# lonelycorn/mvSLAM

Measured on AMD Instinct MI355X. Metric: image-pairs/sec (2k kp, 50k RANSAC hyp), higher is better.
Workload: dtype f64; 1 GPU; 512 independent synthetic 640x480 pairs per GPU, 2000 keypoints (256-bit descriptors), 50000 8-point hypotheses per pair, full match+RANSAC+decompose+triangulate; pairs_per_gpu=512, keypoints=2000, hypotheses=50000, parallelism=pairs sharded, dp1, streams=2

## Files before the change

### mvslam_amd/csrc/kernels.hip

```cpp
#include <algorithm>
#include "kernels.hpp"

#include "device_math.hpp"
#include "prescreen.hpp"

namespace mvs {

constexpr uint32_t kKeyNone = 0xffffffffu;
__device__ __forceinline__ uint32_t bcnt_acc(uint32_t x, uint32_t acc)
{
    uint32_t r;
    asm("v_bcnt_u32_b32 %0, %1, %2" : "=v"(r) : "v"(x), "v"(acc));
    return r;
}
__device__ __forceinline__ void key_insert(uint32_t &k0, uint32_t &k1, uint32_t k)
{
    uint32_t m;
    asm("v_med3_u32 %0, %1, %2, %3" : "=v"(m) : "v"(k0), "v"(k1), "v"(k));
    k1 = m;
    k0 = min(k0, k);
}

constexpr int kTopkWaves = 16;
constexpr int kTopkTileBytes = 65536;
// ... 1422 lines not shown
            a1 = __builtin_amdgcn_mfma_f32_32x32x16_bf16(A0, Bop[1][0], a1, 0, 0, 0);
            a0 = __builtin_amdgcn_mfma_f32_32x32x16_bf16(A1, Bop[0][1], a0, 0, 0, 0);
            a1 = __builtin_amdgcn_mfma_f32_32x32x16_bf16(A1, Bop[1][1], a1, 0, 0, 0);
            ++ntile;
            if (c0 + p0 >= n1) {
#pragma unroll
                for (int r = 0; r < 16; r += 2) {
                    const f32x2 x0 = {a0[r], a0[r + 1]}, x1 = {a1[r], a1[r + 1]};
                    const f32x2 s0 = pk_mul(x0, x0), s1 = pk_mul(x1, x1);
                    cu[0] = pk_add(cu[0], pk_ind(s0, negH, tuH[0]));
                    cl[0] = pk_add(cl[0], pk_ind(s0, negH, tlH[0]));
                    cu[1] = pk_add(cu[1], pk_ind(s1, negH, tuH[1]));
                    cl[1] = pk_add(cl[1], pk_ind(s1, negH, tlH[1]));
                }
            } else {
                dense_count(a0, negH, tlH[0], cl[0]);
                dense_count(a1, negH, tlH[1], cl[1]);
            }
        }
    }
    const int npad = Mr - M;
    int lbest = -1;
#pragma unroll
    for (int c = 0; c < 2; ++c) {
        int U = (int)(cu[c].x + cu[c].y), L = (int)(cl[c].x + cl[c].y);
        U += __shfl_xor(U, 32);
        L += __shfl_xor(L, 32);
        U -= wave_dead ? 0 : npad;
        L -= lpos[c] ? npad : 0;
        if (half == 0 && on[c]) {
            const size_t rec = (size_t)pair * Hp + h[c];
            if (!PILOT)
                b.hyp_cnt[rec] = ucnt0[c] + U;
            if (!wave_dead)
                lbest = max(lbest, L);
        }
        if (STATS && b.stats) {
            const unsigned long long ma = __ballot(wave_live && half == 0);
            if (lane == 0 && ma)
                atomicAdd(&b.stats[PILOT ? 8 : 5], (unsigned long long)__popcll(ma) * (unsigned long long)(32 * ntile));
        }
    }
#pragma unroll
    for (int o = 32; o > 0; o >>= 1)
        lbest = max(lbest, __shfl_xor(lbest, o));
    if (lane == 0 && lbest >= 0)
        atomicMax(&s_lmax, lbest);
    __syncthreads();
    if (tid == 0 && s_lmax >= 0)
        __hip_atomic_fetch_max(b.bound + pair, s_lmax, __ATOMIC_RELAXED, __HIP_MEMORY_SCOPE_AGENT);
}

constexpr int kFinUpperWg = 4;
constexpr int kFinUpperTest = 2;
constexpr int kFinUpperThreads = 512;
constexpr int kFinUpperChunk = 768;
template <bool STATS>
__global__ __launch_bounds__(kFinUpperThreads) __attribute__((amdgpu_waves_per_eu(4, 8))) void ransac_finish_upper_kernel(BatchDev b,
                                                                                                                       RunParams rp)
{
    extern __shared__ __attribute__((aligned(16))) double s_cpts[];
    const int pair = blockIdx.x, tid = threadIdx.x, lane = tid & 63, w = tid >> 6, col = lane & 31, half = lane >> 5;
    const int M = min(b.M[pair], b.max_kp);
    if (M < 8 || b.mode[pair] != 1)
        return;
    const int n1 = b.dense_n1[pair];
    const int Mr = (M + 31) & ~31;
    if (n1 >= Mr)
        return;
    const int Bnow = __hip_atomic_load(b.bound + pair, __ATOMIC_RELAXED, __HIP_MEMORY_SCOPE_AGENT);
    const int cmin = Bnow - (M - n1);
    const int n_all = b.ccount[pair];
    const int n_list = cmin <= 0 ? n_all : min(n_all, b.cpos[(size_t)pair * kSortBins + min(cmin, min(M, kSortBins - 1))]);
    const int n_batches = (max(n_list - kFinishThreads, 0) + kFinUpperThreads - 1) / kFinUpperThreads;
    if ((int)blockIdx.y >= n_batches)
        return;
    const size_t Hp = (size_t)b.max_groups * kHypPerBlock;
    const uint32_t *clist = b.clist2 + (size_t)pair * Hp;
    uint4 *s_op = reinterpret_cast<uint4 *>(s_cpts);
    uint4 *s_win = s_op + (size_t)kFinUpperChunk * 4 + w * kDenseWin;
    const PairBox bx = load_box(b, pair);
    const float X1 = (float)fmax(dabs(bx.x1lo), dabs(bx.x1hi)) * (1.f + 0x1p-22f);
    const float Y1 = (float)fmax(dabs(bx.y1lo), dabs(bx.y1hi)) * (1.f + 0x1p-22f);
    const float X2 = (float)fmax(dabs(bx.x2lo), dabs(bx.x2hi)) * (1.f + 0x1p-22f);
    const float Y2 = (float)fmax(dabs(bx.y2lo), dabs(bx.y2hi)) * (1.f + 0x1p-22f);
    const double4 *src = reinterpret_cast<const double4 *>(b.pts + (size_t)pair * b.max_kp * 4);
    const v16f zero = {0, 0, 0, 0, 0, 0, 0, 0, 0, 0, 0, 0, 0, 0, 0, 0};
    unsigned long long evals = 0;
    struct Ent {
        int h, u;
        bool have;
        float4 q0, q1, q2;
    };
    auto fetch_h = [&](int batch, Ent &en) __attribute__((always_inline)) {
        const int e = kFinishThreads + batch * kFinUpperThreads + w * 64 + lane;
        en.have = batch < n_batches && e < n_list;
        en.h = (int)clist[en.have ? e : 0];
    };
    auto fetch_rest = [&](Ent &en) __attribute__((always_inline)) {
        const size_t rec = (size_t)pair * Hp + (en.have ? en.h : 0);
        en.u = b.hyp_cnt[rec];
        const float4 *fr4 = reinterpret_cast<const float4 *>(b.hyp_r32 + rec * kHypRec32);
        en.q0 = fr4[0], en.q1 = fr4[1], en.q2 = fr4[2];
    };
    for (int c0 = n1; c0 < Mr; c0 += kFinUpperChunk) {
        const int nc = min(kFinUpperChunk, Mr - c0);
        Ent nxt, nn;
        fetch_h(blockIdx.y, nxt);
        fetch_h(blockIdx.y + gridDim.y, nn);
        fetch_rest(nxt);
        __syncthreads();
        for (int i = tid; i < nc; i += kFinUpperThreads) {
            uint4 o[2][2];
            if (c0 + i < M) {
                const double4 pd = src[c0 + i];
                const float x1 = (float)pd.x, y1 = (float)pd.y, x2 = (float)pd.z, y2 = (float)pd.w;
                const float ph[9] = {x2 * x1, x2 * y1, x2, y2 * x1, y2 * y1, y2, x1, y1, 1.f};
                dense_operands_pk<2>(ph, o);
            } else {
                const float qn = __builtin_nanf("");
                const float ph[9] = {qn, qn, qn, qn, qn, qn, qn, qn, qn};
                dense_operands_pk<2>(ph, o);
            }
            uint4 *q = s_op + (size_t)(i >> 5) * 128 + (i & 31);
            q[0] = o[0][0];
            q[32] = o[0][1];
            q[64] = o[1][0];
            q[96] = o[1][1];
        }
        __syncthreads();
        const int left0 = M - c0;
        for (int batch = blockIdx.y; batch < n_batches; batch += gridDim.y) {
            const Ent cur = nxt;
            nxt.have = nn.have;
            nxt.h = nn.h;
            fetch_rest(nxt);
            fetch_h(batch + 2 * gridDim.y, nn);
            const bool have = cur.have;
            const int h_l = cur.have ? cur.h : 0;
            const size_t rec_l = (size_t)pair * Hp + h_l;
            const int u_l = cur.u;
            const bool on_l = have && !(u_l + left0 < Bnow);
            if (__ballot(on_l) == 0ull)
                continue;
            {
                const float4 q0 = cur.q0, q1 = cur.q1, q2 = cur.q2;
                const float fr[9] = {q0.x, q0.y, q0.z, q0.w, q1.x, q1.y, q1.z, q1.w, q2.x};
                float sc = dense_scale(q2.y, dense_T(fr, X1, Y1, X2, Y2), on_l);
                float big = 0.f;
#pragma unroll
                for (int k = 0; k < 9; ++k)
                    big = fmaxf(big, fabsf(fr[k]));
                sc = (big * sc < 0x1p100f) ? sc : 0.f;
                float Fs[9];
#pragma unroll
                for (int k = 0; k < 9; ++k)
                    Fs[k] = mul_legacy(fr[k], sc);
                uint4 o[2][2];
                dense_operands_pk<1>(Fs, o);
                uint4 *wo = s_win + (lane >> 5) * 128 + (lane & 31);
                wo[0] = o[0][0];
                wo[32] = o[0][1];
                wo[64] = o[1][0];
                wo[96] = o[1][1];
            }
            int u0[2];
            bool on[2];
            v8bf Bop[2][2];
#pragma unroll
            for (int c = 0; c < 2; ++c) {
                u0[c] = __shfl(u_l, 32 * c + col);
                on[c] = __shfl((int)on_l, 32 * c + col) != 0;
                const uint4 *ro = s_win + c * 128 + half * 32 + col;
                Bop[c][0] = __builtin_bit_cast(v8bf, ro[0]);
                Bop[c][1] = __builtin_bit_cast(v8bf, ro[64]);
            }
            uint32_t nn[2] = {0u, 0u};
            const uint4 *qt = s_op + half * 32 + col;
            const int nt = nc >> 5;
            int t = 0;
            for (; t < nt; ++t) {
                if (t > 0 && (t & (kFinUpperTest - 1)) == 0) {
                    bool any = false;
#pragma unroll
                    for (int c = 0; c < 2; ++c) {
                        int U = 16 * t - (int)nn[c];
                        U += __shfl_xor(U, 32);
                        any = any || (on[c] && !(u0[c] + U + (left0 - 32 * t) < Bnow));
                    }
                    if (__ballot(any) == 0ull)
                        break;
                }
                const uint4 *q = qt + (size_t)t * 128;
                const v8bf A0 = __builtin_bit_cast(v8bf, q[0]), A1 = __builtin_bit_cast(v8bf, q[64]);
                v16f a0, a1;
                a0 = __builtin_amdgcn_mfma_f32_32x32x16_bf16(A0, Bop[0][0], zero, 0, 0, 0);
                a1 = __builtin_amdgcn_mfma_f32_32x32x16_bf16(A0, Bop[1][0], zero, 0, 0, 0);
                a0 = __builtin_amdgcn_mfma_f32_32x32x16_bf16(A1, Bop[0][1], a0, 0, 0, 0);
                a1 = __builtin_amdgcn_mfma_f32_32x32x16_bf16(A1, Bop[1][1], a1, 0, 0, 0);
                nn[0] += (uint32_t)__builtin_popcount(dense_collect(a0) & 0x55555555u);
                nn[1] += (uint32_t)__builtin_popcount(dense_collect(a1) & 0x55555555u);
            }
            int Uc[2];
#pragma unroll
            for (int c = 0; c < 2; ++c) {
                Uc[c] = 16 * t - (int)nn[c];
                Uc[c] += __shfl_xor(Uc[c], 32);
            }
            const int U1 = __shfl(Uc[1], lane & 31);
            if (on_l)
                b.hyp_cnt[rec_l] = u_l + (lane < 32 ? Uc[0] : U1);
            if (STATS)
                evals += (unsigned long long)__popcll(__ballot(on_l)) * (unsigned long long)(32 * t);
        }
    }
    if (STATS && b.stats && lane == 0 && evals)
        atomicAdd(&b.stats[7], evals);
}

constexpr int kSurvList = 1024;
constexpr int kSurvWg = 8;
__global__ __launch_bounds__(256) void ransac_survivors_kernel(BatchDev b, RunParams rp, int n_active)
{
    __shared__ uint32_t s_x[kSurvList + 1024], s_c[kSurvList + 1024];
    __shared__ int s_nx, s_nc;
    __shared__ unsigned s_bx, s_bc;
    const int pair = blockIdx.y, tid = threadIdx.x, lane = tid & 63;
    if (b.M[pair] < 8)
        return;
    const int mode = b.mode[pair];
    const int bound = b.bound[pair];
    const int H = rp.num_hypotheses;
    const size_t Hp = (size_t)b.max_groups * kHypPerBlock;
    const uint32_t *st4 = reinterpret_cast<const uint32_t *>(b.hyp_okf + (size_t)pair * Hp);
    const int4 *cnt4 = reinterpret_cast<const int4 *>(b.hyp_cnt + (size_t)pair * Hp);
    uint32_t *plist = b.clist + (size_t)pair * Hp;
    if (tid == 0) {
        s_nx = 0;
        s_nc = 0;
    }
    __syncthreads();
    auto flush = [&]() {
        const int nx = s_nx, nc = s_nc;
        if (tid == 0) {
            s_bx = nx ? atomicAdd(&b.xcount[0], (unsigned)nx) : 0u;
            s_bc = nc ? (unsigned)atomicAdd(&b.pcount[pair], nc) : 0u;
        }
        __syncthreads();
        for (int i = tid; i < nx; i += 256)
            b.xlist[s_bx + i] = s_x[i];
        for (int i = tid; i < nc; i += 256)
            plist[s_bc + i] = s_c[i];
        __syncthreads();
        if (tid == 0) {
            s_nx = 0;
            s_nc = 0;
        }
        __syncthreads();
    };
    const int n4 = (int)(Hp / 4);
    const int per_wg = (n4 + gridDim.x - 1) / gridDim.x;
    const int g_begin = blockIdx.x * per_wg, g_end = min(n4, g_begin + per_wg);
    for (int g0 = g_begin; g0 < g_end; g0 += 256) {
        const int g = g0 + tid;
        uint32_t st = 0u;
        int4 c = make_int4(-1, -1, -1, -1);
        if (g < g_end) {
            st = st4[g];
            c = cnt4[g];
        }
        const int cv[4] = {c.x, c.y, c.z, c.w};
#pragma unroll
        for (int k = 0; k < 4; ++k) {
            const int h = 4 * g + k;
            const int okf = (int)((st >> (8 * k)) & 0xffu);
            const bool live = g < g_end && h < H;
            const bool need = live && mode != 0 && (okf == kPsNeedExact || (okf == kPsApprox && cv[k] >= bound));
            const bool cand = need || (live && okf == kPsExact && cv[k] >= bound);
            const unsigned long long mx = __ballot(need), mc = __ballot(cand);
            if (mc) {
                const int first = __builtin_ctzll(mc);
                int bx = 0, bc = 0;
                if (lane == first) {
                    bc = atomicAdd(&s_nc, __popcll(mc));
                    bx = mx ? atomicAdd(&s_nx, __popcll(mx)) : 0;
                }
                bc = __shfl(bc, first);
                bx = __shfl(bx, first);
                if (cand)
                    s_c[bc + __popcll(mc & ((1ull << lane) - 1ull))] = (uint32_t)h;
                if (need)
                    s_x[bx + __popcll(mx & ((1ull << lane) - 1ull))] = (uint32_t)((size_t)pair * Hp + h);
            }
        }
        __syncthreads();
        const bool full = s_nc > kSurvList || s_nx > kSurvList;
        __syncthreads();
        if (full)
            flush();
    }
    flush();
}

constexpr int kSelThreads = 256;
constexpr int kSelList = 2048;
constexpr int kSelWaveCount = 96;
constexpr int kSelSeg = 1024;
constexpr int kSelSerial = 24;

__global__ __launch_bounds__(kSelThreads) void ransac_select_kernel(BatchDev b, RunParams rp, int use_plist)
{
    extern __shared__ __attribute__((aligned(16))) double s_spts[];
    __shared__ uint32_t s_list[kSelList];
    __shared__ int s_cnt[kSelList];
    __shared__ int s_nlist;
    __shared__ double s_F[9];
    __shared__ int s_tot[4];
    __shared__ Cand s_c[4];
    __shared__ Cand s_best;
    __shared__ double s_bestF[9];
    __shared__ uint32_t s_win;
    const int pair = blockIdx.x, tid = threadIdx.x;
    const int M = min(b.M[pair], b.max_kp);
    const int H = rp.num_hypotheses;
    const int G = (H + kHypPerBlock - 1) / kHypPerBlock;
    WgBest *out = b.wgbest + (size_t)pair * b.max_groups;
    for (int g = 1 + tid; g < G; g += kSelThreads) {
        out[g].count = -1;
        out[g].hyp = 0xffffffffu;
        out[g].residual = 0.0;
    }
    if (tid == 0) {
        s_best.cnt = -2;
        s_best.hyp = 0xffffffffu;
        s_best.res = 0.0;
    }
    if (M < 8) {
        if (tid == 0) {
            out[0].count = -1;
            out[0].hyp = 0xffffffffu;
            out[0].residual = 0.0;
        }
        return;
    }
    const size_t Hp = (size_t)b.max_groups * kHypPerBlock;
    const double4 *P4 = reinterpret_cast<const double4 *>(b.pts + (size_t)pair * b.max_kp * 4);
    bool staged = false;
    __syncthreads();
    const int cmax = b.bound[pair];
    const int32_t *cntp = b.hyp_cnt + (size_t)pair * Hp;
    const uint8_t *okb = b.hyp_okf + (size_t)pair * Hp;
    const double *Fp = b.hyp_F + (size_t)pair * Hp * kHypRec;
    const double thr = pair_max_error_sq(b, rp, pair);
    const double4 *L4 = reinterpret_cast<const double4 *>(s_spts);
    double *s_r = s_spts;
    const int lane = tid & 63, w = tid >> 6;
    int scan = 0;
    const int n_total = use_plist ? b.pcount[pair] : H;
    const uint32_t *plist = b.clist + (size_t)pair * Hp;
    while (scan < n_total) {
        if (tid == 0)
            s_nlist = 0;
        __syncthreads();
        if (use_plist) {
            const int n = min(kSelList, n_total - scan);
            for (int q = tid; q < n; q += kSelThreads)
                s_list[q] = plist[scan + q];
            if (tid == 0)
                s_nlist = n;
            scan += n;
            __syncthreads();
        } else {
            while (scan < H) {
                const int seg_end = min(H, scan + kSelSeg);
                for (int h = scan + tid; h < seg_end; h += kSelThreads) {
                    const bool flag = cntp[h] >= cmax && okb[h] != kPsInvalid;
                    const unsigned long long bal = __ballot(flag);
                    if (bal) {
                        int base = 0;
                        if (lane == __builtin_ctzll(bal))
                            base = atomicAdd(&s_nlist, __popcll(bal));
                        base = __shfl(base, __builtin_ctzll(bal));
                        if (flag)
                            s_list[base + __popcll(bal & ((1ull << lane) - 1ull))] = (uint32_t)h;
                    }
                }
                scan = seg_end;
                __syncthreads();
                if (s_nlist > kSelList - kSelSeg)
                    break;
            }
        }
        int n_list = s_nlist;
        __syncthreads();
        if (n_list == 0)
            continue;
        if (b.mode[pair] != 0 && n_list > kSelWaveCount) {
            if (!staged) {
                const double2 *src = reinterpret_cast<const double2 *>(P4);
                double2 *dst = reinterpret_cast<double2 *>(s_spts);
                for (int i = tid; i < 2 * M; i += kSelThreads)
                    dst[i] = src[i];
                staged = true;
                __syncthreads();
            }
            for (int q = tid; q < n_list; q += kSelThreads) {
                const uint32_t h = s_list[q];
                int c = -1;
                if (okb[h] != kPsInvalid) {
                    const double *f = Fp + (size_t)h * kHypRec;
                    double F[9];
#pragma unroll
                    for (int k = 0; k < 9; ++k)
                        F[k] = f[k];
                    c = 0;
#pragma unroll 4
                    for (int i = 0; i < M; ++i) {
                        const double4 p = L4[i];
                        c += epipolar_residual(F, p.x, p.y, p.z, p.w) < thr ? 1 : 0;
                    }
                }
                s_cnt[q] = c;
            }
        } else if (b.mode[pair] != 0) {
            for (int q = w; q < n_list; q += kSelThreads / 64) {
                if (okb[s_list[q]] == kPsInvalid) {
                    if (lane == 0)
                        s_cnt[q] = -1;
                    continue;
                }
                const double *f = Fp + (size_t)s_list[q] * kHypRec;
                double F[9];
#pragma unroll
                for (int k = 0; k < 9; ++k)
                    F[k] = f[k];
                int c = 0;
                for (int i = lane; i < M; i += 64) {
                    const double4 p = P4[i];
                    c += epipolar_residual(F, p.x, p.y, p.z, p.w) < thr ? 1 : 0;
                }
#pragma unroll
                for (int o = 32; o > 0; o >>= 1)
                    c += __shfl_xor(c, o);
                if (lane == 0)
                    s_cnt[q] = c;
            }
        } else {
            for (int q = tid; q < n_list; q += kSelThreads)
                s_cnt[q] = cntp[s_list[q]];
        }
        __syncthreads();
        {
            int cm = -1;
            for (int q = tid; q < n_list; q += kSelThreads)
                cm = max(cm, s_cnt[q]);
#pragma unroll
            for (int o = 32; o > 0; o >>= 1)
                cm = max(cm, __shfl_xor(cm, o));
            if (lane == 0)
                s_tot[w] = cm;
            __syncthreads();
            const int target = max(max(max(s_tot[0], s_tot[1]), max(s_tot[2], s_tot[3])), s_best.cnt);
            __syncthreads();
            int n_ties = 0;
            for (int q0 = 0; q0 < n_list; q0 += kSelThreads) {
                const int q = q0 + tid;
                const bool tie = q < n_list && target >= 0 && s_cnt[q] == target;
                const uint32_t hq = q < n_list ? s_list[q] : 0u;
                const unsigned long long bal = __ballot(tie);
                if (lane == 0)
                    s_tot[w] = __popcll(bal);
                __syncthreads();
                int off = n_ties, tot = 0;
#pragma unroll
                for (int k = 0; k < 4; ++k) {
                    const int v = s_tot[k];
                    off += (k < w) ? v : 0;
                    tot += v;
                }
                if (tie)
                    s_list[off + __popcll(bal & ((1ull << lane) - 1ull))] = hq;
                n_ties += tot;
                __syncthreads();
            }
            n_list = n_ties;
        }
        if (n_list == 0)
            continue;
        if (n_list <= kSelSerial) {
            staged = false;
            for (int q = 0; q < n_list; ++q) {
                const uint32_t h = s_list[q];
                if (tid < 9)
                    s_F[tid] = Fp[(size_t)h * kHypRec + tid];
                __syncthreads();
                double F[9];
#pragma unroll
                for (int k = 0; k < 9; ++k)
                    F[k] = s_F[k];
                int n_in = 0;
                for (int start = 0; start < M; start += kSelThreads) {
                    const int i = start + tid;
                    double r = 0.0;
                    bool in = false;
                    if (i < M) {
                        const double4 p = P4[i];
                        r = epipolar_residual(F, p.x, p.y, p.z, p.w);
                        in = r < thr;
                    }
                    const unsigned long long bal = __ballot(in);
                    if (lane == 0)
                        s_tot[w] = __popcll(bal);
                    __syncthreads();
                    int off = n_in, tot = 0;
#pragma unroll
                    for (int k = 0; k < 4; ++k) {
                        const int v = s_tot[k];
                        off += (k < w) ? v : 0;
                        tot += v;
                    }
                    if (in)
                        s_r[off + __popcll(bal & ((1ull << lane) - 1ull))] = r;
                    n_in += tot;
                    __syncthreads();
                }
                if (tid == 0) {
                    double res = 0.0;
                    int i = 0;
                    for (; i + 8 <= n_in; i += 8) {
                        const double r0 = s_r[i], r1 = s_r[i + 1], r2 = s_r[i + 2], r3 = s_r[i + 3];
                        const double r4 = s_r[i + 4], r5 = s_r[i + 5], r6 = s_r[i + 6], r7 = s_r[i + 7];
                        res += r0; res += r1; res += r2; res += r3;
                        res += r4; res += r5; res += r6; res += r7;
                    }
                    for (; i < n_in; ++i)
                        res += s_r[i];
                    const Cand me{n_in, h, res};
                    if (s_best.cnt < 0 || cand_better(me, s_best)) {
                        s_best = me;
#pragma unroll
                        for (int k = 0; k < 9; ++k)
                            s_bestF[k] = F[k];
                    }
                }
                __syncthreads();
            }
            continue;
        }
        if (!staged) {
            const double2 *src = reinterpret_cast<const double2 *>(P4);
            double2 *dst = reinterpret_cast<double2 *>(s_spts);
            for (int i = tid; i < 2 * M; i += kSelThreads)
                dst[i] = src[i];
            staged = true;
            __syncthreads();
        }
        for (int q0 = 0; q0 < n_list; q0 += kSelThreads) {
            const bool have = q0 + tid < n_list;
            const uint32_t h = have ? s_list[q0 + tid] : 0xffffffffu;
            Cand me{-2, h, 0.0};
            double F[9];
            if (have) {
                const double *f = Fp + (size_t)h * kHypRec;
#pragma unroll
                for (int k = 0; k < 9; ++k)
                    F[k] = f[k];
                int cnt = 0;
                double res = 0.0;
#pragma unroll 4
                for (int i = 0; i < M; ++i) {
                    const double4 p = L4[i];
                    const double r = epipolar_residual(F, p.x, p.y, p.z, p.w);
                    const bool in = r < thr;
                    cnt += in ? 1 : 0;
                    res += in ? r : 0.0;
                }
                me.cnt = cnt;
                me.res = res;
            }
            Cand red = me;
#pragma unroll
            for (int o = 32; o > 0; o >>= 1) {
                Cand other;
                other.cnt = __shfl_xor(red.cnt, o);
                other.hyp = __shfl_xor(red.hyp, o);
                other.res = __shfl_xor(red.res, o);
                if (other.cnt >= 0 && (red.cnt < 0 || cand_better(other, red)))
                    red = other;
            }
            if (lane == 0)
                s_c[w] = red;
            __syncthreads();
            if (tid == 0) {
                Cand best = s_best;
                bool repl = false;
#pragma unroll
                for (int k = 0; k < 4; ++k)
                    if (s_c[k].cnt >= 0 && (best.cnt < 0 || cand_better(s_c[k], best))) {
                        best = s_c[k];
                        repl = true;
                    }
                s_best = best;
                s_win = repl ? best.hyp : 0xfffffffeu;
            }
            __syncthreads();
            if (have && h == s_win) {
#pragma unroll
                for (int k = 0; k < 9; ++k)
                    s_bestF[k] = F[k];
            }
            __syncthreads();
        }
    }
    if (tid == 0) {
        const Cand best = s_best;
        out[0].count = best.cnt >= 0 ? best.cnt : -1;
        out[0].hyp = best.cnt >= 0 ? best.hyp : 0xffffffffu;
        out[0].residual = best.cnt >= 0 ? best.res : 0.0;
        if (best.cnt >= 0) {
#pragma unroll
            for (int k = 0; k < 9; ++k)
                out[0].F[k] = s_bestF[k];
        }
    }
}


__global__ __launch_bounds__(64, 1) void fundamental_kernel(const double *p1, const double *p2, double *Fout, int *okout)
{
    if (threadIdx.x != 0)
        return;
    double x1[8], y1[8], x2[8], y2[8], F[9];
#pragma unroll
    for (int k = 0; k < 8; ++k) {
        x1[k] = p1[2 * k]; y1[k] = p1[2 * k + 1];
        x2[k] = p2[2 * k]; y2[k] = p2[2 * k + 1];
    }
    unsigned rot = 0, pairs = 0;
    bool bad = false;
    bool ok = eight_point<Solve::GuardedCheap>(x1, y1, x2, y2, F, rot, pairs, bad);
    if (bad)
        ok = eight_point<Solve::Ieee>(x1, y1, x2, y2, F, rot, pairs, bad);
#pragma unroll
    for (int k = 0; k < 9; ++k)
        Fout[k] = F[k];
    *okout = ok ? 1 : 0;
}

constexpr int kFinThreads = 256;

template <typename Pred, typename Emit>
__device__ __forceinline__ int block_compact(int n, int *s_tot, Pred pred, Emit emit)
{
    const int tid = threadIdx.x, lane = tid & 63, w = tid >> 6;
    int basepos = 0;
    for (int start = 0; start < n; start += kFinThreads) {
        const int i = start + tid;
        const bool flag = (i < n) && pred(i);
        const unsigned long long bal = __ballot(flag);
        const int pre = __popcll(bal & ((1ull << lane) - 1ull));
        if (lane == 0)
            s_tot[w] = __popcll(bal);
        __syncthreads();
        int off = basepos, tot = 0;
#pragma unroll
        for (int k = 0; k < 4; ++k) {
            const int v = s_tot[k];
            off += (k < w) ? v : 0;
            tot += v;
        }
        if (flag)
            emit(i, off + pre);
        basepos += tot;
        __syncthreads();
    }
    return basepos;
}

__device__ __forceinline__ void triangulate_item(const BatchDev &b, int pair, int c, int j, const double *R, const double *Rr,
                                                 double t0, double t1, double t2)
{
    const size_t base = (size_t)pair * b.max_kp;
    const int i = b.inl[base + j];
    const double4 p = *reinterpret_cast<const double4 *>(b.pts + (base + i) * 4);
    double At[4][4];
    auto design = [&]() {
        At[0][0] = -1.0; At[1][0] = 0.0;  At[2][0] = p.x; At[3][0] = 0.0;
        At[0][1] = 0.0;  At[1][1] = -1.0; At[2][1] = p.y; At[3][1] = 0.0;
        At[0][2] = p.z * Rr[6] - Rr[0]; At[1][2] = p.z * Rr[7] - Rr[1]; At[2][2] = p.z * Rr[8] - Rr[2]; At[3][2] = p.z * t2 - t0;
        At[0][3] = p.w * Rr[6] - Rr[3]; At[1][3] = p.w * Rr[7] - Rr[4]; At[2][3] = p.w * Rr[8] - Rr[5]; At[3][3] = p.w * t2 - t1;
    };
    double X[4];
    unsigned rot = 0, prs = 0;
    bool bad = false;
    design();
    svd4_last_vt_row<true>(At, X, rot, prs, bad);
    if (__builtin_expect(__any(bad), 0)) {
        design();
        svd4_last_vt_row<false>(At, X, rot, prs, bad);
    }
    bool okp = !(dabs(X[3]) < kTol);
    const double scale = 1.0 / X[3];
    const double px = X[0] * scale, py = X[1] * scale, pz = X[2] * scale;
    okp = okp && !(pz < kTol);
    const double z2 = ((R[6] * px + R[7] * py) + R[8] * pz) + t2;
    okp = okp && !(z2 < kTol);
    b.okf[((size_t)pair * 4 + c) * b.max_kp + j] = okp ? 1 : 0;
    double *dst = b.cand_pts + (((size_t)pair * 4 + c) * b.max_kp + j) * 3;
    dst[0] = px; dst[1] = py; dst[2] = pz;
}

__global__ __launch_bounds__(kFinThreads) void finalize_model_kernel(BatchDev b, RunParams rp, int mode)
{
    __shared__ double s_F[9], s_E[9];
    __shared__ int s_tot[4];
    __shared__ int s_proceed;
    __shared__ Cand s_red[4];
    __shared__ uint32_t s_grp[4];
    const int pair = blockIdx.x, tid = threadIdx.x;
    const size_t base = (size_t)pair * b.max_kp;
    const int M = min(b.M[pair], b.max_kp);
    mvs_pair_result *res = b.results + pair;
    FinModel *fm = b.fin + pair;
    const double *P = b.pts + base * 4;
    uint8_t *mask = b.mask + base;

    if (tid == 0)
        s_proceed = 0;
    __syncthreads();

    if (mode == kFinalizeFull) {
        const int G = (rp.num_hypotheses + kHypPerBlock - 1) / kHypPerBlock;
        Cand me{-2, 0xffffffffu, 0.0};
        uint32_t mygroup = 0;
        if (M >= 8) {
            const WgBest *wb = b.wgbest + (size_t)pair * b.max_groups;
            for (int g = tid; g < G; g += kFinThreads) {
                Cand c{wb[g].count, wb[g].hyp, wb[g].residual};
                if (c.cnt >= 0 && (me.cnt < -1 || cand_better(c, me))) {
                    me = c;
                    mygroup = g;
                }
            }
        }
#pragma unroll
        for (int o = 32; o > 0; o >>= 1) {
            Cand other;
            other.cnt = __shfl_xor(me.cnt, o);
            other.hyp = __shfl_xor(me.hyp, o);
            other.res = __shfl_xor(me.res, o);
            const uint32_t og = __shfl_xor(mygroup, o);
            if (other.cnt >= 0 && (me.cnt < -1 || cand_better(other, me))) {
                me = other;
                mygroup = og;
            }
        }
        if ((tid & 63) == 0) {
            s_red[tid >> 6] = me;
            s_grp[tid >> 6] = mygroup;
        }
        __syncthreads();
        if (tid == 0) {
            Cand best = s_red[0];
            uint32_t bg = s_grp[0];
            for (int w = 1; w < 4; ++w)
                if (s_red[w].cnt >= 0 && (best.cnt < -1 || cand_better(s_red[w], best))) {
                    best = s_red[w];
                    bg = s_grp[w];
                }
            res->valid = 0;
            res->n_matches = M;
            res->n_inliers = 0;
            res->n_points = 0;
            res->best_hyp = best.cnt >= 0 ? (int)best.hyp : -1;
            res->best_count = best.cnt >= 0 ? best.cnt : 0;
            res->best_residual = best.cnt >= 0 ? best.res : 0.0;
            if (best.cnt >= 0) {
                const WgBest *wb = b.wgbest + (size_t)pair * b.max_groups + bg;
#pragma unroll
                for (int k = 0; k < 9; ++k) {
                    s_F[k] = wb->F[k];
                    res->F[k] = wb->F[k];
                }
                s_proceed = 1;
            }
        }
        __syncthreads();
        for (int i = M + tid; i < b.max_kp; i += kFinThreads)
            mask[i] = 0;
        if (!s_proceed) {
            for (int i = tid; i < M; i += kFinThreads)
                mask[i] = 0;
            if (tid == 0) {
                fm->proceed = 0;
                fm->n_inl = 0;
                fm->ncand = 0;
            }
            return;
        }
        double F[9];
#pragma unroll
        for (int k = 0; k < 9; ++k)
            F[k] = s_F[k];
        const double thr = pair_max_error_sq(b, rp, pair);
        for (int i = tid; i < M; i += kFinThreads) {
            const double4 p = *reinterpret_cast<const double4 *>(P + (size_t)i * 4);
            mask[i] = epipolar_residual(F, p.x, p.y, p.z, p.w) < thr ? 1 : 0;
        }
        __syncthreads();
    } else if (tid == 0) {
        res->valid = 0;
        res->n_matches = M;
        res->n_points = 0;
        if (mode != kFinalizeEssential) {
            res->best_hyp = -1;
            res->best_count = 0;
            res->best_residual = 0.0;
        }
    }

    uint16_t *inl = b.inl + base;
    const int n_inl = block_compact(
        M, s_tot, [&](int i) { return mask[i] != 0; }, [&](int i, int pos) { inl[pos] = (uint16_t)i; });

    if (tid == 0) {
        res->n_inliers = n_inl;
        unsigned rot = 0, prs = 0;
        bool go = true;
        int ncand = 4;
        if (mode == kFinalizeFull) {
            double Fm[3][3], w[3], U[3][3], Vt[3][3];
#pragma unroll
            for (int i = 0; i < 3; ++i)
#pragma unroll
                for (int j = 0; j < 3; ++j)
                    Fm[i][j] = s_F[i * 3 + j];
            svd3_full(Fm, w, U, Vt, rot, prs);
            const double v = dsqrt(w[0] * w[1]);
#pragma unroll
            for (int i = 0; i < 3; ++i) {
                const double a = U[i][0] * v, c = U[i][1] * v;
#pragma unroll
                for (int j = 0; j < 3; ++j) {
                    const double e = a * Vt[0][j] + c * Vt[1][j];
                    s_E[i * 3 + j] = e;
                    res->E[i * 3 + j] = e;
                }
            }
            go = (res->best_count > 0) && (n_inl >= rp.min_inliers);
        } else if (mode == kFinalizeFromE || mode == kFinalizeEssential) {
#pragma unroll
            for (int k = 0; k < 9; ++k)
                s_E[k] = res->E[k];
            if (mode == kFinalizeEssential)
                go = (res->best_count > 0) && (n_inl >= rp.min_inliers);
        }
        if (mode == kFinalizeTriangulate) {
            double R[3][3];
#pragma unroll
            for (int i = 0; i < 3; ++i)
#pragma unroll
                for (int j = 0; j < 3; ++j) {
                    R[i][j] = res->R1to2[i * 3 + j];
                    fm->R[0][i * 3 + j] = R[i][j];
                }
            rectify3(R);
#pragma unroll
            for (int i = 0; i < 3; ++i)
#pragma unroll
                for (int j = 0; j < 3; ++j)
                    fm->Rr[0][i * 3 + j] = R[i][j];
#pragma unroll
            for (int k = 0; k < 3; ++k)
                fm->T[k] = res->t1to2[k];
            ncand = 1;
        } else if (go) {
            double Em[3][3], w[3], U[3][3], Vt[3][3], V[3][3];
#pragma unroll
            for (int i = 0; i < 3; ++i)
#pragma unroll
                for (int j = 0; j < 3; ++j)
                    Em[i][j] = s_E[i * 3 + j];
            svd3_full(Em, w, U, Vt, rot, prs);
#pragma unroll
            for (int i = 0; i < 3; ++i)
#pragma unroll
                for (int j = 0; j < 3; ++j)
                    V[i][j] = Vt[j][i];
            if (det3(U) < 0.0) {
#pragma unroll
                for (int i = 0; i < 3; ++i)
#pragma unroll
                    for (int j = 0; j < 3; ++j)
                        U[i][j] = -U[i][j];
            }
            if (det3(V) < 0.0) {
#pragma unroll
                for (int i = 0; i < 3; ++i)
#pragma unroll
                    for (int j = 0; j < 3; ++j)
// ... 634 lines not shown
```

Baseline: 115,700 pairs/s.

## Widen RANSAC select block and parallelize inlier counting over points

Raises the select kernel's block size from 256 to 1024 threads and generalizes the per-wave reductions to the new wave count. In the mode!=0 path, each thread now owns a point and loops over the candidate hypotheses, whose F matrices are staged in shared memory. Per-hypothesis inlier counts are accumulated with wave ballots and shared atomics, replacing the old scheme of one wave per hypothesis. The larger block may lower occupancy and adds atomic contention and ballot overhead per hypothesis. The s_Fl buffer holds kSelWaveCount*9 entries, so it overflows if n_list exceeds kSelWaveCount.

After: 116,200 pairs/s, median of 6. Within noise of the previous version (+0.4%).

```diff
diff --git a/mvslam_amd/csrc/kernels.hip b/mvslam_amd/csrc/kernels.hip
--- a/mvslam_amd/csrc/kernels.hip
+++ b/mvslam_amd/csrc/kernels.hip
@@ -1748,7 +1748,8 @@
     flush();
 }
 
-constexpr int kSelThreads = 256;
+constexpr int kSelThreads = 1024;
+constexpr int kSelWaves = kSelThreads / 64;
 constexpr int kSelList = 2048;
 constexpr int kSelWaveCount = 96;
 constexpr int kSelSeg = 1024;
@@ -1761,8 +1762,9 @@
     __shared__ int s_cnt[kSelList];
     __shared__ int s_nlist;
     __shared__ double s_F[9];
-    __shared__ int s_tot[4];
-    __shared__ Cand s_c[4];
+    __shared__ double s_Fl[kSelWaveCount * 9];
+    __shared__ int s_tot[kSelWaves];
+    __shared__ Cand s_c[kSelWaves];
     __shared__ Cand s_best;
     __shared__ double s_bestF[9];
     __shared__ uint32_t s_win;
@@ -1869,27 +1871,27 @@
                 s_cnt[q] = c;
             }
         } else if (b.mode[pair] != 0) {
-            for (int q = w; q < n_list; q += kSelThreads / 64) {
-                if (okb[s_list[q]] == kPsInvalid) {
-                    if (lane == 0)
-                        s_cnt[q] = -1;
-                    continue;
+            for (int q = tid; q < n_list; q += kSelThreads)
+                s_cnt[q] = okb[s_list[q]] == kPsInvalid ? -1 : 0;
+            for (int k = tid; k < n_list * 9; k += kSelThreads)
+                s_Fl[k] = Fp[(size_t)s_list[k / 9] * kHypRec + (k % 9)];
+            __syncthreads();
+            for (int start = 0; start < M; start += kSelThreads) {
+                const int i = start + tid;
+                const bool have = i < M;
+                const double4 p = have ? P4[i] : make_double4(0.0, 0.0, 0.0, 0.0);
+                for (int q = 0; q < n_list; ++q) {
+                    if (s_cnt[q] < 0)
+                        continue;
+                    double F[9];
+#pragma unroll
+                    for (int k = 0; k < 9; ++k)
+                        F[k] = s_Fl[q * 9 + k];
+                    const bool in = have && epipolar_residual(F, p.x, p.y, p.z, p.w) < thr;
+                    const unsigned long long bal = __ballot(in);
+                    if (lane == 0 && bal)
+                        atomicAdd(&s_cnt[q], __popcll(bal));
                 }
-                const double *f = Fp + (size_t)s_list[q] * kHypRec;
-                double F[9];
-#pragma unroll
-                for (int k = 0; k < 9; ++k)
-                    F[k] = f[k];
-                int c = 0;
-                for (int i = lane; i < M; i += 64) {
-                    const double4 p = P4[i];
-                    c += epipolar_residual(F, p.x, p.y, p.z, p.w) < thr ? 1 : 0;
-                }
-#pragma unroll
-                for (int o = 32; o > 0; o >>= 1)
-                    c += __shfl_xor(c, o);
-                if (lane == 0)
-                    s_cnt[q] = c;
             }
         } else {
             for (int q = tid; q < n_list; q += kSelThreads)
@@ -1906,7 +1908,10 @@
             if (lane == 0)
                 s_tot[w] = cm;
             __syncthreads();
-            const int target = max(max(max(s_tot[0], s_tot[1]), max(s_tot[2], s_tot[3])), s_best.cnt);
+            int target = s_best.cnt;
+#pragma unroll
+            for (int k = 0; k < kSelWaves; ++k)
+                target = max(target, s_tot[k]);
             __syncthreads();
             int n_ties = 0;
             for (int q0 = 0; q0 < n_list; q0 += kSelThreads) {
@@ -1919,7 +1924,7 @@
                 __syncthreads();
                 int off = n_ties, tot = 0;
 #pragma unroll
-                for (int k = 0; k < 4; ++k) {
+                for (int k = 0; k < kSelWaves; ++k) {
                     const int v = s_tot[k];
                     off += (k < w) ? v : 0;
                     tot += v;
@@ -1960,7 +1965,7 @@
                     __syncthreads();
                     int off = n_in, tot = 0;
 #pragma unroll
-                    for (int k = 0; k < 4; ++k) {
+                    for (int k = 0; k < kSelWaves; ++k) {
                         const int v = s_tot[k];
                         off += (k < w) ? v : 0;
                         tot += v;
@@ -2041,7 +2046,7 @@
                 Cand best = s_best;
                 bool repl = false;
 #pragma unroll
-                for (int k = 0; k < 4; ++k)
+                for (int k = 0; k < kSelWaves; ++k)
                     if (s_c[k].cnt >= 0 && (best.cnt < 0 || cand_better(s_c[k], best))) {
                         best = s_c[k];
                         repl = true;
```
